# Fuad-HH/PumiUMTally

Hardware: AMD Instinct MI355X
Metric: particle-steps/sec (higher is better)
Workload: dtype fp64; 1 GPU; model=track-length-tally-walk, mesh_tets=998250, global_batch=10000000, particles_per_gpu=10000000, parallelism=dp1-replicated-mesh, nscores=1, comm=torch-rccl, ngroups=1, device=gpu, lost_particles=0

## Files before the change

### cpp/origin_delta_bench.cpp

```cpp
#include "core/origin_delta.h"

#include <hip/hip_runtime.h>

#include <algorithm>
#include <chrono>
#include <cstdio>
#include <cstdlib>
#include <cstring>
#include <memory>
#include <random>
#include <vector>

using namespace pumitally;

static double *pinned_doubles(int64_t count) {
  void *p = nullptr;
  if (hipHostMalloc(&p, count * sizeof(double), hipHostMallocDefault) !=
      hipSuccess) {
    std::fprintf(stderr, "hipHostMalloc failed\n");
    std::exit(2);
  }
  return (double *)p;
}

// ... 3 lines not shown
  double *ends[2] = {pinned_doubles(n * 3), pinned_doubles(n * 3)};
  double *alt = pinned_doubles(n * 3);
  std::mt19937_64 rng(1);
  std::uniform_real_distribution<double> u(0.0, 1.0);
  for (int64_t k = 0; k < n * 3; ++k) {
    ends[0][k] = u(rng);
    ends[1][k] = u(rng);
  }
  std::memcpy(alt, ends[0], n * 3 * sizeof(double));
  for (int64_t i = 0; i < n; ++i)
    if (rng() % 10 == 0) alt[i * 3 + 1] = u(rng);
  std::unique_ptr<double[]> shadow(new double[n * 3]);
  int64_t cap = 0;
  for (int nt : {1, 4, 8, 16})
    cap = std::max(cap, origin_delta_patch_capacity(n, nt));
  void *pi = nullptr, *px = nullptr;
  if (hipHostMalloc(&pi, cap * sizeof(int32_t), hipHostMallocDefault) !=
          hipSuccess ||
      hipHostMalloc(&px, cap * 3 * sizeof(double), hipHostMallocDefault) !=
          hipSuccess) {
    std::fprintf(stderr, "hipHostMalloc failed\n");
    return 2;
  }
  std::printf("n=%lld reps=%d (96 B/particle streamed, 120 B ordinary)\n",
              (long long)n, reps);
  for (int nt : {1, 4, 8, 16}) {
    OriginDeltaPool pool(nt);
    for (int nontemporal = 1; nontemporal >= 0; --nontemporal) {
      for (int frac10 = 0; frac10 < 2; ++frac10) {
        origin_delta_seed(pool, ends[0], shadow.get(), 0, n, nontemporal != 0);
        std::vector<double> ms;
        int64_t changed = 0;
        for (int r = 0; r < reps; ++r) {
          const double *origin =
              (frac10 && (r & 1) == 0) ? alt : ends[r & 1];
          const auto t0 = std::chrono::steady_clock::now();
          OriginDeltaResult res = origin_delta_pass(
              pool, origin, ends[(r + 1) & 1], shadow.get(), 0, n,
              (int32_t *)pi, (double *)px, nontemporal != 0);
          if (!res.overflow)
            origin_delta_compact(res, (int32_t *)pi, (double *)px);
          const auto t1 = std::chrono::steady_clock::now();
          ms.push_back(std::chrono::duration<double, std::milli>(t1 - t0)
                           .count());
          changed += res.changed;
        }
        std::sort(ms.begin(), ms.end());
        std::printf("threads=%2d stores=%-9s changed=%-4s  min %7.2f ms  "
                    "median %7.2f ms  (%.1f GB/s at median; changed/pass "
                    "%lld)\n",
                    nt, nontemporal ? "streaming" : "ordinary",
                    frac10 ? "~5%" : "0", ms.front(), ms[ms.size() / 2],
                    (nontemporal ? 96.0 : 120.0) * n / ms[ms.size() / 2] / 1e6,
                    (long long)(changed / reps));
      }
    }
  }
  return 0;
}
```

### csrc/core/engine.h

```cpp
#pragma once

#include "mesh.h"
#include "walk.h"

#include <cstdint>
#include <cstdlib>
#include <stdexcept>
#include <memory>
#include <string>
#include <vector>

namespace pumitally {

struct EngineStats {
  int64_t lost_particles = 0;
  int64_t moves = 0;
  int64_t relocated = 0;
  int64_t loose_localizations = 0;
  int64_t origins_elided = 0;
  int64_t origin_bytes_uploaded = 0;
  double origin_pass_seconds = 0.0;
  int64_t collisions_scored = 0;
  int64_t collision_misses = 0;
  int64_t tracks = 0;
  int64_t track_entries = 0;
  int64_t track_misses = 0;
};

constexpr int kMaxLostRecords = 16;

class Engine {
public:
  virtual ~Engine() = default;

  virtual int64_t num_particles() const = 0;
  virtual const Mesh &mesh() const = 0;

  virtual void copy_initial_position(const double *positions, int64_t n) = 0;

  virtual void move(const double *origin, const double *dest,
                    const int8_t *flying, const double *weights, int64_t n,
                    const uint16_t *groups = nullptr,
                    const double *responses = nullptr) = 0;

// ... 142 lines not shown
  };
  virtual bool device_mesh(DeviceMeshView *out) const {
    (void)out;
    return false;
  }

  int max_steps = 0;
  int ngroups = 1;
  int nscores = 1;

  bool reflective = false;

  bool linear = false;

  bool face_currents = false;

  bool collision_tallies = false;

  bool walk_fp32 = false;

  bool origin_elide = true;
  int origin_threads = 8;
  int64_t origin_chunk = 0;

protected:
  [[noreturn]] static void throw_not_linear() {
    throw std::runtime_error(
        "linear moment tallies are off: create the engine with linear=true");
  }
  [[noreturn]] static void throw_not_currents() {
    throw std::runtime_error(
        "face-current tallies are off: create the engine with currents=true");
  }
  [[noreturn]] static void throw_not_collisions() {
    throw std::runtime_error(
        "collision tallies are off: create the engine with collisions=true");
  }
};

inline bool default_walk_fp32() {
  const char *s = getenv("PUMITALLY_WALK");
  return s && std::string(s) == "fp32";
}

inline bool default_origin_elide() {
  const char *s = getenv("PUMITALLY_ORIGIN_ELIDE");
  return !s || atoi(s) != 0;
}

inline int default_origin_threads() {
  const char *s = getenv("PUMITALLY_ORIGIN_THREADS");
  const int k = s ? atoi(s) : 8;
  return k < 1 ? 1 : (k > 16 ? 16 : k);
}

inline int64_t default_origin_chunk() {
  const char *s = getenv("PUMITALLY_ORIGIN_CHUNK");
  const int64_t c = s ? (int64_t)atoll(s) : 0;
  return c < 0 ? 0 : c;
}

inline bool default_reflective() {
  const char *s = getenv("PUMITALLY_BC");
  return s && std::string(s) == "reflective";
}

inline double loc_tol_rel() {
  const char *s = getenv("PUMITALLY_LOC_TOL");
  return s ? atof(s) : 1e-10;
}
// ... 28 lines not shown
```

### csrc/core/origin_delta.cpp

```cpp
#include "origin_delta.h"

#include <algorithm>
#include <atomic>
#include <cstring>

#if defined(__SSE2__) && !defined(__HIP_DEVICE_COMPILE__)
#include <emmintrin.h>
#define PT_HAVE_STREAM_STORE 1
#else
#define PT_HAVE_STREAM_STORE 0
#endif

namespace pumitally {

int origin_delta_clamp_threads(int requested) {
  return std::max(1, std::min(requested, kOriginDeltaMaxThreads));
}

OriginDeltaPool::OriginDeltaPool(int nthreads)
    : nthreads_(origin_delta_clamp_threads(nthreads)) {
  for (int t = 1; t < nthreads_; ++t)
    threads_.emplace_back([this, t] { worker(t); });
}

// ... 90 lines not shown
        pidx[count] = (int32_t)i;
        pxyz[count * 3] = o[0];
        pxyz[count * 3 + 1] = o[1];
        pxyz[count * 3 + 2] = o[2];
      }
      ++count;
    }
    const double *d = dest + i * 3;
    store_bits<NT>(s, load_bits(d));
    store_bits<NT>(s + 1, load_bits(d + 1));
    store_bits<NT>(s + 2, load_bits(d + 2));
  }
  if (NT) store_fence();
  return count;
}

template <bool NT>
void copy_part(const double *dest, double *shadow, int64_t lo, int64_t hi) {
  for (int64_t k = lo * 3; k < hi * 3; ++k)
    store_bits<NT>(shadow + k, load_bits(dest + k));
  if (NT) store_fence();
}

}

int64_t origin_delta_block(int64_t len, int nthreads) {
  const int64_t t = origin_delta_clamp_threads(nthreads);
  const int64_t b = (len + 4 * t - 1) / (4 * t);
  return std::max<int64_t>(1, std::min(b, kMaxBlock));
}

int64_t origin_delta_patch_capacity(int64_t len, int nthreads) {
  if (len <= 0) return 0;
  const int64_t block = origin_delta_block(len, nthreads);
  const int64_t full = len / block, tail = len % block;
  return full * seg_capacity(block) + (tail ? seg_capacity(tail) : 0);
}

OriginDeltaResult origin_delta_pass(OriginDeltaPool &pool,
                                    const double *origin, const double *dest,
                                    double *shadow, int64_t lo, int64_t hi,
                                    int32_t *patch_idx, double *patch_xyz,
                                    bool nontemporal) {
  OriginDeltaResult r;
  const int64_t len = hi - lo;
  if (len <= 0) return r;
  r.block = origin_delta_block(len, pool.nthreads());
  r.nsegs = (len + r.block - 1) / r.block;
  r.seg_off.resize(r.nsegs);
  r.seg_cap.resize(r.nsegs);
  r.seg_count.assign(r.nsegs, 0);
  for (int64_t b = 0; b < r.nsegs; ++b) {
    const int64_t blen = std::min(r.block, len - b * r.block);
    r.seg_off[b] = b * seg_capacity(r.block);
    r.seg_cap[b] = seg_capacity(blen);
  }
  std::atomic<int64_t> next{0};
  const std::function<void(int)> job = [&](int) {
    for (;;) {
      const int64_t b = next.fetch_add(1, std::memory_order_relaxed);
      if (b >= r.nsegs) return;
      const int64_t a = lo + b * r.block;
      const int64_t e = std::min(hi, a + r.block);
      int32_t *pi = patch_idx + r.seg_off[b];
      double *px = patch_xyz + r.seg_off[b] * 3;
      r.seg_count[b] =
          nontemporal
              ? delta_part<true>(origin, dest, shadow, a, e, pi, px,
                                 r.seg_cap[b])
              : delta_part<false>(origin, dest, shadow, a, e, pi, px,
                                  r.seg_cap[b]);
    }
  };
  pool.run(job);
  for (int64_t b = 0; b < r.nsegs; ++b) {
    r.changed += r.seg_count[b];
    if (r.seg_count[b] > r.seg_cap[b]) r.overflow = true;
  }
  return r;
}

void origin_delta_compact(const OriginDeltaResult &r, int32_t *patch_idx,
                          double *patch_xyz) {
  int64_t out = 0;
  for (int64_t b = 0; b < r.nsegs; ++b) {
    const int64_t cnt = r.seg_count[b];
    if (cnt && r.seg_off[b] != out) {
      std::memmove(patch_idx + out, patch_idx + r.seg_off[b],
                   cnt * sizeof(int32_t));
      std::memmove(patch_xyz + out * 3, patch_xyz + r.seg_off[b] * 3,
                   cnt * 3 * sizeof(double));
    }
    out += cnt;
  }
}

void origin_delta_seed(OriginDeltaPool &pool, const double *dest,
                       double *shadow, int64_t lo, int64_t hi,
                       bool nontemporal) {
  const int64_t len = hi - lo;
  if (len <= 0) return;
// ... 20 lines not shown
```

### csrc/core/origin_delta.h

```cpp
#pragma once

#include <condition_variable>
#include <cstdint>
#include <functional>
#include <mutex>
#include <thread>
#include <vector>

namespace pumitally {

constexpr int kOriginDeltaMaxThreads = 16;

int origin_delta_clamp_threads(int requested);

class OriginDeltaPool {
public:
  explicit OriginDeltaPool(int nthreads);
  ~OriginDeltaPool();
  OriginDeltaPool(const OriginDeltaPool &) = delete;
  OriginDeltaPool &operator=(const OriginDeltaPool &) = delete;

  int nthreads() const { return nthreads_; }
  void run(const std::function<void(int)> &f);

// ... 9 lines not shown
  int pending_ = 0;
  bool stop_ = false;
};

struct OriginDeltaResult {
  int64_t block = 0;
  int64_t nsegs = 0;
  std::vector<int64_t> seg_off, seg_cap;
  std::vector<int64_t> seg_count;
  int64_t changed = 0;
  bool overflow = false;
};

int64_t origin_delta_block(int64_t len, int nthreads);

int64_t origin_delta_patch_capacity(int64_t len, int nthreads);

OriginDeltaResult origin_delta_pass(OriginDeltaPool &pool,
                                    const double *origin, const double *dest,
                                    double *shadow, int64_t lo, int64_t hi,
                                    int32_t *patch_idx, double *patch_xyz,
                                    bool nontemporal = false);

void origin_delta_compact(const OriginDeltaResult &r, int32_t *patch_idx,
                          double *patch_xyz);

void origin_delta_seed(OriginDeltaPool &pool, const double *dest,
                       double *shadow, int64_t lo, int64_t hi,
                       bool nontemporal = false);

}
```

### csrc/hip/engine_gpu.hip

```cpp
#include "../core/engine.h"
#include "../core/origin_delta.h"
#include "../core/tally_sink.h"
#include "../core/track.h"
#include "../core/walk.h"
#include "hip_util.h"

#include <hip/hip_runtime.h>
#include <hipcub/hipcub.hpp>

#include <algorithm>
#include <type_traits>
#include <array>
#include <chrono>
#include <cstdio>
#include <cstdlib>
#include <cstring>
#include <memory>
#include <stdexcept>
#include <string>
#include <vector>

namespace pumitally {

namespace {
// ... 670 lines not shown

int grid_blocks(int64_t work) {
  int64_t blocks = (work + kBlock - 1) / kBlock;
  if (blocks > grid_cap()) blocks = grid_cap();
  return (int)((blocks + 7) / 8 * 8);
}

class GpuEngine final : public Engine {
public:
  GpuEngine(Mesh mesh, int64_t n, int device, int groups, int scores,
            bool lin, bool cur, bool coll)
      : mesh_(std::move(mesh)), n_(n) {
    ngroups = groups < 1 ? 1 : groups;
    nscores = scores < 1 ? 1 : scores;
    linear = lin;
    face_currents = cur;
    collision_tallies = coll;
    PT_HIP_CHECK(hipSetDevice(device));
    device_ = device;
    s_copy_.create();
    s_comp_.create();
    for (auto &ev : copy_ev_) ev.create();
    for (auto &ev : kernels_done_) ev.create();
    if (collision_tallies) {
      s_score_.create();
      score_copied_.create();
      score_done_.create();
    }

    d_planes_ = upload(mesh_.planes);
    d_planes32_ = upload(mesh_.planes32);
    d_nbr_ = upload(mesh_.nbr);
    d_cell_start_ = upload(mesh_.grid.cell_start);
    d_cell_tets_.allocate(mesh_.grid.cell_tets.size() + 1);
    PT_HIP_CHECK(hipMemcpy(d_cell_tets_, mesh_.grid.cell_tets.data(),
                           mesh_.grid.cell_tets.size() * sizeof(int32_t),
                           hipMemcpyHostToDevice));
    d_face_bc_ = upload(mesh_.face_bc_bits);
    if (mesh_.has_periodic()) {
      d_pidx_ = upload(mesh_.periodic_idx);
      d_pelem_ = upload(mesh_.periodic_elem);
      d_pshift_ = upload(mesh_.periodic_shift);
    }
    grid_view_ = GridView{mesh_.grid.nx, mesh_.grid.ny, mesh_.grid.nz,
                          mesh_.grid.lo,  mesh_.grid.inv_h,
                          d_cell_start_,  d_cell_tets_};
// ... 13 lines not shown
      mesh_.build_inv_heights();
      d_inv_h_ = upload(mesh_.inv_heights);
      d_moments_.allocate(fsz_ * 4);
      PT_HIP_CHECK(hipMemset(d_moments_, 0, fsz_ * 4 * sizeof(double)));
    }
    if (face_currents) {
      d_cur_.allocate(fsz_ * 4);
      PT_HIP_CHECK(hipMemset(d_cur_, 0, fsz_ * 4 * sizeof(double)));
      cur_keyed_ = currents_keyed_agg() && mesh_.nelems < ((int64_t)1 << 29);
    }
    if (collision_tallies) {
      d_coll_.allocate(fsz_);
      PT_HIP_CHECK(hipMemset(d_coll_, 0, fsz_ * sizeof(double)));
      d_coll_counts_.allocate(2);
      PT_HIP_CHECK(
          hipMemset(d_coll_counts_, 0, 2 * sizeof(unsigned long long)));
      coll_agg_ = collisions_run_agg();
    }
    PT_HIP_CHECK(hipMemset(d_lost_, 0, sizeof(unsigned long long)));
    PT_HIP_CHECK(hipMemset(d_loose_, 0, sizeof(unsigned long long)));
    PT_HIP_CHECK(
        hipMemset(d_lostrec_, 0, kMaxLostRecords * 4 * sizeof(double)));

    for (int p = 0; p < 2; ++p) {
      d_origin_[p].allocate(n_ * 3);
      d_dest_[p].allocate(n_ * 3);
      d_flying_[p].allocate(n_);
      d_weights_[p].allocate(n_);
      if (ngroups > 1) d_groups_[p].allocate(n_);
    }

    sort_every_ = sort_every();
    if (sort_every_ > 0) {
      d_keys_.allocate(n_);
      d_keys2_.allocate(n_);
      d_vals_.allocate(n_);
      d_order_.allocate(n_);
      d_pos2_.allocate(n_ * 3);
      d_elem2_.allocate(n_);
      d_esc2_.allocate(n_);
      d_s2c2_.allocate(n_);
      size_t bytes = 0;
      PT_HIP_CHECK(hipcub::DeviceRadixSort::SortPairs(
          nullptr, bytes, d_keys_.get(), d_keys2_.get(), d_vals_.get(),
          d_order_.get(), (int)n_, 0, 64, s_comp_));
      sorttmp_bytes_ = bytes;
      d_sorttmp_.allocate(bytes ? bytes : 1);
      const Vec3 ext = mesh_.bbox_hi - mesh_.bbox_lo;
      sort_scale_ = Vec3{ext.x > 0 ? 2097151.0 / ext.x : 0.0,
                         ext.y > 0 ? 2097151.0 / ext.y : 0.0,
                         ext.z > 0 ? 2097151.0 / ext.z : 0.0};
    }

    loc_tol_ = loc_tol_rel() * norm(mesh_.bbox_hi - mesh_.bbox_lo);
    walk_fp32 = default_walk_fp32();
    reflective = default_reflective();
    origin_elide = default_origin_elide();
    origin_threads = default_origin_threads();
    origin_chunk = default_origin_chunk();
    const Vec3 c0 = mesh_.nelems > 0 ? mesh_.centroid(0) : Vec3{0, 0, 0};
    k_init_particles<<<grid_blocks(n_), kBlock, 0, s_comp_>>>(
        d_pos_, d_elem_, d_escaped_, d_s2c_, n_, c0.x, c0.y, c0.z);
    PT_HIP_CHECK(hipGetLastError());
    PT_HIP_CHECK(hipStreamSynchronize(s_comp_));
  }

  ~GpuEngine() override {
    (void)hipSetDevice(device_);
    (void)hipDeviceSynchronize();
  }

  int64_t num_particles() const override { return n_; }
  const Mesh &mesh() const override { return mesh_; }

  void copy_initial_position(const double *p, int64_t n) override {
    check_n(n);
    PT_HIP_CHECK(hipSetDevice(device_));
    sync();
    stage(p, n * 3 * sizeof(double), d_origin_[0], s_copy_);
    PT_HIP_CHECK(hipStreamSynchronize(s_copy_));
    k_iota<<<grid_blocks(n_), kBlock, 0, s_comp_>>>(d_s2c_, n_);
    k_locate<<<grid_blocks(n_), kBlock, 0, s_comp_>>>(
        d_planes_, grid_view_, d_origin_[0], d_pos_, d_elem_, d_escaped_,
        d_loose_, n_, loc_tol_);
    PT_HIP_CHECK(hipGetLastError());
    if (sort_every_ > 0) spatial_sort();
    moves_since_sort_ = 0;
    PT_HIP_CHECK(hipStreamSynchronize(s_comp_));
  }

  void move(const double *origin, const double *dest, const int8_t *flying,
            const double *weights, int64_t n,
            const uint16_t *groups = nullptr,
            const double *responses = nullptr) override {
    check_n(n);
    PT_HIP_CHECK(hipSetDevice(device_));
    const int steps = max_steps > 0 ? max_steps : default_max_steps(mesh_);
    const int p = (int)(parity_++ & 1);
    PT_HIP_CHECK(hipStreamWaitEvent(s_copy_, kernels_done_[p], 0));
    if (responses && !d_resp_[p]) d_resp_[p].allocate(n_ * nscores);
    const bool probe = origin && origin_elide && n > 0 && elide_skip_ == 0;
    if (probe && shadow_valid_) {
      stage_elided(p, origin, dest, flying, weights, groups, responses, n);
    } else {
      if (origin) {
        stage(origin, n * 3 * sizeof(double), d_origin_[p], s_copy_);
        stats_.origin_bytes_uploaded += n * 3 * (int64_t)sizeof(double);
      }
      stage_inputs(p, dest, flying, weights, groups, responses, n);
      shadow_valid_ = false;
      if (probe) {
        ensure_elide_host(n);
        const auto t0 = std::chrono::steady_clock::now();
        origin_delta_seed(*delta_pool_, dest, shadow_.get(), 0, n,
                          false);
        stats_.origin_pass_seconds += seconds_since(t0);
        shadow_valid_ = true;
      } else if (origin && origin_elide && elide_skip_ > 0) {
        --elide_skip_;
      }
    }
    PT_HIP_CHECK(hipEventRecord(copy_ev_[p], s_copy_));
    PT_HIP_CHECK(hipStreamWaitEvent(s_comp_, copy_ev_[p], 0));
    launch_move_chunks(origin ? d_origin_[p] : nullptr, d_dest_[p],
                       d_flying_[p], d_weights_[p],
                       groups ? d_groups_[p] : nullptr,
                       responses ? d_resp_[p] : nullptr, n, steps);
    PT_HIP_CHECK(hipEventRecord(kernels_done_[p], s_comp_));
    maybe_resort();
    PT_HIP_CHECK(hipStreamSynchronize(s_copy_));
    stats_.moves++;
  }

  void move_device(const double *d_origin, const double *d_dest,
                   const int8_t *d_flying, const double *d_weights, int64_t n,
                   const uint16_t *d_groups = nullptr,
                   const double *d_responses = nullptr) override {
    check_n(n);
    PT_HIP_CHECK(hipSetDevice(device_));
    const int steps = max_steps > 0 ? max_steps : default_max_steps(mesh_);
    launch_move_chunks(d_origin, d_dest, d_flying, d_weights, d_groups,
                       d_responses, n, steps);
    maybe_resort();
    stats_.moves++;
  }

  void score_collisions(const int8_t *active, const double *weights,
                        int64_t n, const uint16_t *groups = nullptr,
                        const double *responses = nullptr) override {
    if (!collision_tallies) throw_not_collisions();
    check_n(n);
// ... 497 lines not shown
    PT_HIP_CHECK(hipMemcpy(d_elem_, elem, n * sizeof(int32_t), hipMemcpyHostToDevice));
    PT_HIP_CHECK(hipMemcpy(d_escaped_, escaped, n, hipMemcpyHostToDevice));
    moves_since_sort_ = sort_every_;
  }

  void synchronize() override { sync(); }

  bool device_mesh(DeviceMeshView *out) const override {
    out->planes = d_planes_;
    out->nbr = d_nbr_;
    out->grid = grid_view_;
    out->stream = (void *)s_comp_;
    return true;
  }

private:
  void check_n(int64_t n) const {
    if (n != n_) throw std::runtime_error("particle count mismatch");
  }

  void sync() const {
    PT_HIP_CHECK(hipStreamSynchronize(s_copy_));
    PT_HIP_CHECK(hipStreamSynchronize(s_comp_));
  }

  void stage(const void *src, size_t bytes, void *dst, hipStream_t s) {
    PT_HIP_CHECK(hipMemcpyAsync(dst, src, bytes, hipMemcpyHostToDevice, s));
  }

  void stage_inputs(int p, const double *dest, const int8_t *flying,
                    const double *weights, const uint16_t *groups,
                    const double *responses, int64_t n) {
    stage(dest, n * 3 * sizeof(double), d_dest_[p], s_copy_);
    stage(flying, n * sizeof(int8_t), d_flying_[p], s_copy_);
    stage(weights, n * sizeof(double), d_weights_[p], s_copy_);
    if (groups && d_groups_[p])
      stage(groups, n * sizeof(uint16_t), d_groups_[p], s_copy_);
    if (responses)
      stage(responses, n * nscores * sizeof(double), d_resp_[p], s_copy_);
  }

  static constexpr int kElideBackoffFirst = 16;
  static constexpr int kElideBackoffMax = 256;

  static double seconds_since(std::chrono::steady_clock::time_point t0) {
    return std::chrono::duration<double>(std::chrono::steady_clock::now() -
                                         t0)
        .count();
  }

  int64_t elide_chunk(int64_t n) const {
    if (origin_chunk > 0) return std::max<int64_t>(origin_chunk, 64);
    return std::max<int64_t>((int64_t)262144, (n + 1) / 2);
  }

  void ensure_elide_host(int64_t n) {
    const int want = origin_delta_clamp_threads(origin_threads);
    if (!delta_pool_ || delta_pool_->nthreads() != want)
      delta_pool_ = std::make_unique<OriginDeltaPool>(want);
    if (!shadow_) shadow_.reset(new double[n * 3]);
  }

  void ensure_patch(int64_t need) {
    if (need <= patch_cap_) return;
    PT_HIP_CHECK(hipStreamSynchronize(s_copy_));
    patch_cap_ = 0;
    h_patch_idx_.reset();
    h_patch_xyz_.reset();
    d_patch_idx_.reset();
    d_patch_xyz_.reset();
    h_patch_idx_.allocate(need);
    h_patch_xyz_.allocate(need * 3);
    d_patch_idx_.allocate(need);
    d_patch_xyz_.allocate(need * 3);
    patch_cap_ = need;
  }

  void stage_elided(int p, const double *origin, const double *dest,
                    const int8_t *flying, const double *weights,
                    const uint16_t *groups, const double *responses,
                    int64_t n) {
    ensure_elide_host(n);
    const int nthreads = delta_pool_->nthreads();
    const int64_t chunk = elide_chunk(n);
    int64_t need = 0;
    for (int64_t lo = 0; lo < n; lo += chunk)
      need += origin_delta_patch_capacity(std::min(chunk, n - lo), nthreads);
    ensure_patch(need);
    shadow_valid_ = false;
    k_copy_doubles<<<grid_blocks(n * 3 / 2), kBlock, 0, s_copy_>>>(
        d_dest_[p ^ 1], d_origin_[p], n * 3);
    PT_HIP_CHECK(hipGetLastError());
    stage_inputs(p, dest, flying, weights, groups, responses, n);
    int64_t region = 0, uploaded = 0;
    for (int64_t lo = 0; lo < n; lo += chunk) {
      const int64_t hi = std::min(n, lo + chunk);
      const int64_t len = hi - lo;
      const int64_t cap = origin_delta_patch_capacity(len, nthreads);
      if (region + cap > patch_cap_)
        throw std::runtime_error("origin elision: patch region overflow");
      int32_t *hidx = h_patch_idx_ + region;
      double *hxyz = h_patch_xyz_ + region * 3;
      const auto t0 = std::chrono::steady_clock::now();
      const OriginDeltaResult r = origin_delta_pass(
          *delta_pool_, origin, dest, shadow_.get(), lo, hi, hidx, hxyz,
          false);
      stats_.origin_pass_seconds += seconds_since(t0);
      if (r.overflow || r.changed * 2 > len) {
        stage(origin + lo * 3, len * 3 * sizeof(double),
              d_origin_[p] + lo * 3, s_copy_);
        uploaded += len;
      } else if (r.changed > 0) {
        origin_delta_compact(r, hidx, hxyz);
        stage(hidx, r.changed * sizeof(int32_t), d_patch_idx_ + region,
              s_copy_);
        stage(hxyz, r.changed * 3 * sizeof(double),
              d_patch_xyz_ + region * 3, s_copy_);
        k_scatter_origins<<<grid_blocks(r.changed), kBlock, 0, s_copy_>>>(
            d_patch_idx_ + region, d_patch_xyz_ + region * 3, d_origin_[p],
            r.changed);
        PT_HIP_CHECK(hipGetLastError());
        uploaded += r.changed;
      }
      region += cap;
    }
    stats_.origins_elided += n - uploaded;
    stats_.origin_bytes_uploaded += uploaded * 3 * (int64_t)sizeof(double);
    shadow_valid_ = true;
    if (uploaded * 2 > n) {
      elide_skip_ = elide_backoff_;
      elide_backoff_ = std::min(elide_backoff_ * 2, kElideBackoffMax);
    } else {
      elide_backoff_ = kElideBackoffFirst;
    }
  }

  void launch_walk_raw(int64_t n, const double *pos, const double *dest,
                       const int32_t *elem, const double *weights,
                       double *out_pos, int32_t *out_elem, int8_t *out_status,
                       const uint16_t *groups, const double *resp,
                       double *out_dest, const double *in_t,
                       const int32_t *in_prev, double *out_o, double *out_t,
                       int32_t *out_prev) {
    const int steps = max_steps > 0 ? max_steps : default_max_steps(mesh_);
    const auto kernel =
        linear ? (walk_fp32 ? k_walk_raw<true, true> : k_walk_raw<false, true>)
        : face_currents
            ? (walk_fp32 ? k_walk_raw<true, false, true>
                         : k_walk_raw<false, false, true>)
            : (walk_fp32 ? k_walk_raw<true> : k_walk_raw<false>);
    kernel<<<grid_blocks(n), kBlock, 0, s_comp_>>>(
        d_planes_, d_planes32_, d_nbr_, pos, dest, elem, weights, groups, resp,
        out_pos, out_elem, out_status, out_dest, d_flux_, d_lost_, d_lostrec_,
        n, steps, reflective, d_face_bc_, ngroups, mesh_.nelems, nscores,
        d_pidx_, d_pelem_, d_pshift_, in_t, in_prev, out_o, out_t, out_prev,
        d_inv_h_, d_moments_, d_cur_);
    PT_HIP_CHECK(hipGetLastError());
// ... 68 lines not shown

  template <class T>
  std::pair<std::vector<int32_t>, std::vector<T>> fetch(const T *dev,
                                                        int comps) const {
    sync();
    std::vector<int32_t> s2c(n_);
    std::vector<T> v(n_ * comps);
    PT_HIP_CHECK(hipMemcpy(s2c.data(), d_s2c_, n_ * sizeof(int32_t),
                           hipMemcpyDeviceToHost));
    PT_HIP_CHECK(hipMemcpy(v.data(), dev, n_ * comps * sizeof(T),
                           hipMemcpyDeviceToHost));
    return {std::move(s2c), std::move(v)};
  }

  Mesh mesh_;
  int64_t n_;
  int64_t fsz_ = 0;
  int device_ = 0;
  double loc_tol_ = 1e-12;
  int slices_ = 1;
  int sort_every_ = 0;
  int64_t moves_since_sort_ = 0;
  uint64_t parity_ = 0;
  Vec3 sort_scale_{0, 0, 0};

  std::unique_ptr<double[]> shadow_;
  bool shadow_valid_ = false;
  std::unique_ptr<OriginDeltaPool> delta_pool_;
  int64_t patch_cap_ = 0;
  int elide_skip_ = 0;
  int elide_backoff_ = kElideBackoffFirst;

  Stream s_copy_, s_comp_;
  std::array<Event, 2> copy_ev_;
  std::array<Event, 2> kernels_done_;
  Stream s_score_;
  Event score_copied_, score_done_;
  bool score_queued_ = false;

  PinnedBuffer<int32_t> h_patch_idx_;
  PinnedBuffer<double> h_patch_xyz_;
  DeviceBuffer<int32_t> d_patch_idx_;
  DeviceBuffer<double> d_patch_xyz_;

  DeviceBuffer<Plane> d_planes_;
  DeviceBuffer<Plane32> d_planes32_;
  DeviceBuffer<int32_t> d_nbr_, d_cell_start_, d_cell_tets_;
  GridView grid_view_{};

  DeviceBuffer<double> d_pos_;
  DeviceBuffer<int32_t> d_elem_;
  DeviceBuffer<uint8_t> d_escaped_;
  DeviceBuffer<int32_t> d_s2c_;
  DeviceBuffer<double> d_flux_;
  DeviceBuffer<unsigned long long> d_lost_, d_loose_;
  DeviceBuffer<double> d_lostrec_;
  DeviceBuffer<double> d_origin_[2], d_dest_[2], d_weights_[2], d_resp_[2];
  DeviceBuffer<int8_t> d_flying_[2];
  DeviceBuffer<uint16_t> d_groups_[2];
  DeviceBuffer<double> d_bsum_, d_bsq_;
  DeviceBuffer<double> d_inv_h_, d_moments_, d_msum_;
  DeviceBuffer<double> d_cur_, d_csum_, d_csq_;
  bool cur_keyed_ = false;
  DeviceBuffer<double> d_coll_, d_collsum_, d_collsq_;
  DeviceBuffer<unsigned long long> d_coll_counts_;
  bool coll_agg_ = true;
  DeviceBuffer<int8_t> sc_active_;
  DeviceBuffer<double> sc_weights_, sc_resp_;
  DeviceBuffer<uint16_t> sc_groups_;
  ScorePointsScratch sp_;
  DeviceBuffer<uint32_t> d_face_bc_;
  DeviceBuffer<int32_t> d_pidx_, d_pelem_;
  DeviceBuffer<double> d_pshift_;
  WalkRawScratch wr_;
  DeviceBuffer<int32_t> d_face_start_, d_face_list_;
  DeviceBuffer<unsigned long long> d_track_counts_;
  bool tracks_refused_ = false;
  TrackScratch tt_;
  int64_t nbatches_ = 0;

// ... 31 lines not shown
```

### csrc/pybind/module.cpp

```cpp
#include <pybind11/numpy.h>
#include <pybind11/pybind11.h>
#include <pybind11/stl.h>

#include "../api/PumiTally.h"
#include "../comm/comm.h"
#include "../core/engine.h"
#include "../core/partition_engine.h"

#include <hip/hip_runtime.h>

#include <cstdint>
#include <cstring>
#include <memory>
#include <thread>
#include <vector>

namespace py = pybind11;
using namespace pumitally;

namespace {

bool have_gpu() {
  int n = 0;
  if (hipGetDeviceCount(&n) != hipSuccess) {
// ... 683 lines not shown
          [](const PyEngine &e) { return e.eng->face_currents; })
      .def_property_readonly(
          "reflective", [](const PyEngine &e) { return e.eng->reflective; })
      .def_property_readonly("ngroups",
                             [](const PyEngine &e) { return e.eng->ngroups; })
      .def_property_readonly("nscores",
                             [](const PyEngine &e) { return e.eng->nscores; })
      .def_property_readonly("num_particles",
                             [](const PyEngine &e) { return e.eng->num_particles(); })
      .def_property_readonly("is_gpu", [](const PyEngine &e) { return e.gpu; })
      .def_property(
          "max_steps", [](const PyEngine &e) { return e.eng->max_steps; },
          [](PyEngine &e, int v) { e.eng->max_steps = v; })
      .def_property(
          "origin_elide", [](const PyEngine &e) { return e.eng->origin_elide; },
          [](PyEngine &e, bool v) { e.eng->origin_elide = v; })
      .def_property(
          "origin_threads",
          [](const PyEngine &e) { return e.eng->origin_threads; },
          [](PyEngine &e, int v) { e.eng->origin_threads = v; })
      .def_property(
          "origin_chunk", [](const PyEngine &e) { return e.eng->origin_chunk; },
          [](PyEngine &e, int64_t v) { e.eng->origin_chunk = v; })
      .def("copy_initial_position",
           [](PyEngine &e, py::array_t<double, py::array::c_style | py::array::forcecast> p) {
             if ((int64_t)p.size() != e.eng->num_particles() * 3)
               throw std::runtime_error("positions must have size 3*num_particles");
             e.eng->copy_initial_position(p.data(), e.eng->num_particles());
           })
      .def("move",
           [](PyEngine &e, py::array_t<double, py::array::c_style> origin,
              py::array_t<double, py::array::c_style> dest,
              py::array_t<int8_t, py::array::c_style> flying,
              py::array_t<double, py::array::c_style> weights,
              py::object groups, py::object responses) {
             const int64_t n = e.eng->num_particles();
             if ((int64_t)origin.size() != n * 3 || (int64_t)dest.size() != n * 3 ||
                 (int64_t)flying.size() != n || (int64_t)weights.size() != n)
               throw std::runtime_error("move: array size mismatch");
             const uint16_t *gp = nullptr;
             py::array_t<uint16_t, py::array::c_style | py::array::forcecast> garr;
             if (!groups.is_none()) {
               garr = groups.cast<py::array_t<uint16_t, py::array::c_style | py::array::forcecast>>();
               if ((int64_t)garr.size() != n)
                 throw std::runtime_error("move: groups size mismatch");
               gp = garr.data();
// ... 303 lines not shown
              py::array_t<int32_t, py::array::c_style | py::array::forcecast> elem,
              py::array_t<uint8_t, py::array::c_style | py::array::forcecast> escaped) {
             const int64_t n = e.eng->num_particles();
             if ((int64_t)pos.size() != n * 3 || (int64_t)elem.size() != n ||
                 (int64_t)escaped.size() != n)
               throw std::runtime_error("set_particle_state: size mismatch");
             e.eng->set_particle_state(pos.data(), elem.data(), escaped.data(), n);
           })
      .def("end_batch", [](PyEngine &e) { py::gil_scoped_release ng; e.eng->end_batch(); })
      .def("batch_sum", [](const PyEngine &e) { return vec_to_np(e.eng->batch_sum()); })
      .def("batch_sum_sq", [](const PyEngine &e) { return vec_to_np(e.eng->batch_sum_sq()); })
      .def_property_readonly("num_batches",
                             [](const PyEngine &e) { return e.eng->num_batches(); })
      .def("stats", [](const PyEngine &e) {
        const EngineStats &s = e.eng->stats();
        py::dict d;
        d["lost_particles"] = s.lost_particles;
        d["moves"] = s.moves;
        d["relocated"] = s.relocated;
        d["loose_localizations"] = s.loose_localizations;
        d["origins_elided"] = s.origins_elided;
        d["origin_bytes_uploaded"] = s.origin_bytes_uploaded;
        d["origin_pass_seconds"] = s.origin_pass_seconds;
        d["collisions_scored"] = s.collisions_scored;
        d["collision_misses"] = s.collision_misses;
        d["tracks"] = s.tracks;
        d["track_entries"] = s.track_entries;
        d["track_misses"] = s.track_misses;
        return d;
      })
      .def("lost_records", [](const PyEngine &e) {
        auto v = e.eng->lost_records();
        auto arr = vec_to_np(std::move(v));
        return arr.reshape({(py::ssize_t)(arr.size() / 4), (py::ssize_t)4});
      });

  py::class_<PumiTally>(m, "PumiTally")
      .def(py::init([](const std::string &mesh, int32_t n) {
        int argc = 0;
        char **argv = nullptr;
        return new PumiTally(mesh, n, argc, argv);
      }))
      .def("copy_initial_position",
           [](PumiTally &t, py::array_t<double, py::array::c_style | py::array::forcecast> p) {
             t.CopyInitialPosition((double *)p.data(), (int32_t)p.size());
           })
// ... 19 lines not shown
```

### pumiumtally_amd/__init__.py

```python
from __future__ import annotations

import os as _os

if _os.environ.get("PUMITALLY_NO_TORCH", "0") != "1":
    try:
        import torch as _torch
    except ImportError:
        pass


def _load_core():
    try:
        from . import _core
        return _core
    except ImportError as e:
        if _os.environ.get("PUMITALLY_AUTOBUILD", "1") == "1":
            from ._build import build
            build()
            from . import _core
            return _core
        raise ImportError(
            "pumiumtally_amd._core is not built. Run "
            "`python -m pumiumtally_amd._build` first."
        ) from e
# ... 84 lines not shown
    @property
    def origin_elide(self) -> bool:
        return self._eng.origin_elide

    @origin_elide.setter
    def origin_elide(self, v: bool) -> None:
        self._eng.origin_elide = bool(v)

    @property
    def origin_threads(self) -> int:
        return self._eng.origin_threads

    @origin_threads.setter
    def origin_threads(self, v: int) -> None:
        self._eng.origin_threads = int(v)

    @property
    def origin_chunk(self) -> int:
        return self._eng.origin_chunk

    @origin_chunk.setter
    def origin_chunk(self, v: int) -> None:
        self._eng.origin_chunk = int(v)

    def copy_initial_position(self, positions):
        self._eng.copy_initial_position(positions)

    def move(self, origin, dest, flying, weights, groups=None,
             responses=None):
        self._eng.move(origin, dest, flying, weights, groups, responses)

    def move_continue(self, dest, flying, weights, groups=None,
                      responses=None):
        self._eng.move_continue(dest, flying, weights, groups, responses)

    def move_from_device(self, dest, flying, weights, origin=None,
                         sync_torch=True, groups=None, responses=None):
        def ptr(t, dtype, numel):
            return _device_ptr(t, dtype, numel, "move_from_device")

        n = self.num_particles
        if sync_torch:
            _sync_torch()
        self._eng.move_device(
            ptr(origin, "<f8", n * 3), ptr(dest, "<f8", n * 3),
            ptr(flying, "|i1", n), ptr(weights, "<f8", n),
# ... 432 lines not shown
```

Before: 1.445 billion particle-steps/s.

## Skip origin copy kernel when unchanged; add echo and owned-block origin elision modes

Rotates three device dest buffers so that, when no origin patches are needed, the walk reads origins in place from the previous step's dest buffer instead of launching a device copy kernel. It also adds two opt-in modes. One echoes device dest back to pinned host memory in slices and compares against it, so the host shadow copy write is dropped. The other uses owned-block work stealing for the host delta pass. The default path gains the copy-skip and extra buffer rotation, at the cost of an extra n*3 device buffer and more event synchronisation.

```diff
diff --git a/cpp/origin_delta_bench.cpp b/cpp/origin_delta_bench.cpp
--- a/cpp/origin_delta_bench.cpp
+++ b/cpp/origin_delta_bench.cpp
@@ -49,37 +49,63 @@
     std::fprintf(stderr, "hipHostMalloc failed\n");
     return 2;
   }
-  std::printf("n=%lld reps=%d (96 B/particle streamed, 120 B ordinary)\n",
+  std::printf("n=%lld reps=%d (96 B/particle streamed, 120 B ordinary, 48 B "
+              "compare only)\n",
               (long long)n, reps);
+  double *echoed = pinned_doubles(n * 3);
   for (int nt : {1, 4, 8, 16}) {
     OriginDeltaPool pool(nt);
-    for (int nontemporal = 1; nontemporal >= 0; --nontemporal) {
-      for (int frac10 = 0; frac10 < 2; ++frac10) {
-        origin_delta_seed(pool, ends[0], shadow.get(), 0, n, nontemporal != 0);
-        std::vector<double> ms;
-        int64_t changed = 0;
-        for (int r = 0; r < reps; ++r) {
-          const double *origin =
-              (frac10 && (r & 1) == 0) ? alt : ends[r & 1];
-          const auto t0 = std::chrono::steady_clock::now();
-          OriginDeltaResult res = origin_delta_pass(
-              pool, origin, ends[(r + 1) & 1], shadow.get(), 0, n,
-              (int32_t *)pi, (double *)px, nontemporal != 0);
-          if (!res.overflow)
-            origin_delta_compact(res, (int32_t *)pi, (double *)px);
-          const auto t1 = std::chrono::steady_clock::now();
-          ms.push_back(std::chrono::duration<double, std::milli>(t1 - t0)
-                           .count());
-          changed += res.changed;
+    for (int pass = 0; pass < 3; ++pass) {
+      for (int nontemporal = (pass == 0 ? 1 : 0); nontemporal >= 0;
+           --nontemporal) {
+        for (int frac10 = 0; frac10 < 2; ++frac10) {
+          if (pass == 1)
+            origin_delta_seed_owned(pool, ends[0], shadow.get(), 0, n);
+          else if (pass == 0)
+            origin_delta_seed(pool, ends[0], shadow.get(), 0, n,
+                              nontemporal != 0);
+          std::vector<double> ms;
+          int64_t changed = 0;
+          for (int r = 0; r < reps; ++r) {
+            const double *origin =
+                (frac10 && (r & 1) == 0) ? alt : ends[r & 1];
+            const double *dest = ends[(r + 1) & 1];
+            if (pass == 2)
+              std::memcpy(echoed, ends[r & 1], n * 3 * sizeof(double));
+            const auto t0 = std::chrono::steady_clock::now();
+            OriginDeltaResult res =
+                pass == 2   ? origin_delta_compare(pool, origin, echoed, 0, n,
+                                                   (int32_t *)pi, (double *)px)
+                : pass == 1 ? origin_delta_pass_owned(
+                                  pool, origin, dest, shadow.get(), 0, n,
+                                  (int32_t *)pi, (double *)px)
+                            : origin_delta_pass(
+                                  pool, origin, dest, shadow.get(), 0, n,
+                                  (int32_t *)pi, (double *)px,
+                                  nontemporal != 0);
+            if (!res.overflow)
+              origin_delta_compact(res, (int32_t *)pi, (double *)px);
+            const auto t1 = std::chrono::steady_clock::now();
+            ms.push_back(
+                std::chrono::duration<double, std::milli>(t1 - t0).count());
+            changed += res.changed;
+          }
+          std::sort(ms.begin(), ms.end());
+          const double bytes = pass == 2 ? 48.0 : nontemporal ? 96.0 : 120.0;
+          std::printf("threads=%2d pass=%-7s stores=%-9s changed=%-4s  min "
+                      "%7.2f ms  median %7.2f ms  (%.1f GB/s at median; "
+                      "changed/pass %lld)\n",
+                      nt,
+                      pass == 2   ? "compare"
+                      : pass == 1 ? "owned"
+                                  : "shared",
+                      pass == 2     ? "none"
+                      : nontemporal ? "streaming"
+                                    : "ordinary",
+                      frac10 ? "~5%" : "0", ms.front(), ms[ms.size() / 2],
+                      bytes * n / ms[ms.size() / 2] / 1e6,
+                      (long long)(changed / reps));
         }
-        std::sort(ms.begin(), ms.end());
-        std::printf("threads=%2d stores=%-9s changed=%-4s  min %7.2f ms  "
-                    "median %7.2f ms  (%.1f GB/s at median; changed/pass "
-                    "%lld)\n",
-                    nt, nontemporal ? "streaming" : "ordinary",
-                    frac10 ? "~5%" : "0", ms.front(), ms[ms.size() / 2],
-                    (nontemporal ? 96.0 : 120.0) * n / ms[ms.size() / 2] / 1e6,
-                    (long long)(changed / reps));
       }
     }
   }
diff --git a/csrc/core/engine.h b/csrc/core/engine.h
--- a/csrc/core/engine.h
+++ b/csrc/core/engine.h
@@ -20,6 +20,8 @@
   int64_t origins_elided = 0;
   int64_t origin_bytes_uploaded = 0;
   double origin_pass_seconds = 0.0;
+  int64_t origin_copy_kernels = 0;
+  double origin_echo_wait_seconds = 0.0;
   int64_t collisions_scored = 0;
   int64_t collision_misses = 0;
   int64_t tracks = 0;
@@ -208,6 +210,9 @@
   bool origin_elide = true;
   int origin_threads = 8;
   int64_t origin_chunk = 0;
+  bool origin_echo = false;
+  int origin_slices = 4;
+  bool origin_owned = false;
 
 protected:
   [[noreturn]] static void throw_not_linear() {
@@ -232,6 +237,22 @@
 inline bool default_origin_elide() {
   const char *s = getenv("PUMITALLY_ORIGIN_ELIDE");
   return !s || atoi(s) != 0;
+}
+
+inline bool default_origin_echo() {
+  const char *s = getenv("PUMITALLY_ORIGIN_ECHO");
+  return s && atoi(s) != 0;
+}
+
+inline bool default_origin_owned() {
+  const char *s = getenv("PUMITALLY_ORIGIN_OWNED");
+  return s && atoi(s) != 0;
+}
+
+inline int default_origin_slices() {
+  const char *s = getenv("PUMITALLY_ORIGIN_SLICES");
+  const int k = s ? atoi(s) : 4;
+  return k < 1 ? 1 : (k > 8 ? 8 : k);
 }
 
 inline int default_origin_threads() {
diff --git a/csrc/core/origin_delta.cpp b/csrc/core/origin_delta.cpp
--- a/csrc/core/origin_delta.cpp
+++ b/csrc/core/origin_delta.cpp
@@ -136,30 +136,44 @@
   if (NT) store_fence();
 }
 
-}
-
-int64_t origin_delta_block(int64_t len, int nthreads) {
-  const int64_t t = origin_delta_clamp_threads(nthreads);
-  const int64_t b = (len + 4 * t - 1) / (4 * t);
-  return std::max<int64_t>(1, std::min(b, kMaxBlock));
-}
-
-int64_t origin_delta_patch_capacity(int64_t len, int nthreads) {
-  if (len <= 0) return 0;
-  const int64_t block = origin_delta_block(len, nthreads);
-  const int64_t full = len / block, tail = len % block;
-  return full * seg_capacity(block) + (tail ? seg_capacity(tail) : 0);
-}
-
-OriginDeltaResult origin_delta_pass(OriginDeltaPool &pool,
-                                    const double *origin, const double *dest,
-                                    double *shadow, int64_t lo, int64_t hi,
-                                    int32_t *patch_idx, double *patch_xyz,
-                                    bool nontemporal) {
+constexpr int64_t kCompareTile = 64;
+
+inline uint64_t xor_or(const double *a, const double *b, int64_t nw) {
+  uint64_t acc = 0;
+  for (int64_t k = 0; k < nw; ++k) acc |= load_bits(a + k) ^ load_bits(b + k);
+  return acc;
+}
+
+int64_t compare_part(const double *origin, const double *shadow, int64_t lo,
+                     int64_t hi, int32_t *pidx, double *pxyz, int64_t cap) {
+  int64_t count = 0;
+  for (int64_t t = lo; t < hi; t += kCompareTile) {
+    const int64_t te = std::min(hi, t + kCompareTile);
+    if (!xor_or(origin + t * 3, shadow + t * 3, (te - t) * 3)) continue;
+    for (int64_t i = t; i < te; ++i) {
+      const double *o = origin + i * 3;
+      const double *s = shadow + i * 3;
+      const uint64_t diff = (load_bits(o) ^ load_bits(s)) |
+                            (load_bits(o + 1) ^ load_bits(s + 1)) |
+                            (load_bits(o + 2) ^ load_bits(s + 2));
+      if (diff) {
+        if (count < cap) {
+          pidx[count] = (int32_t)i;
+          pxyz[count * 3] = o[0];
+          pxyz[count * 3 + 1] = o[1];
+          pxyz[count * 3 + 2] = o[2];
+        }
+        ++count;
+      }
+    }
+  }
+  return count;
+}
+
+OriginDeltaResult segment_layout(int64_t len, int nthreads) {
   OriginDeltaResult r;
-  const int64_t len = hi - lo;
   if (len <= 0) return r;
-  r.block = origin_delta_block(len, pool.nthreads());
+  r.block = origin_delta_block(len, nthreads);
   r.nsegs = (len + r.block - 1) / r.block;
   r.seg_off.resize(r.nsegs);
   r.seg_cap.resize(r.nsegs);
@@ -169,6 +183,63 @@
     r.seg_off[b] = b * seg_capacity(r.block);
     r.seg_cap[b] = seg_capacity(blen);
   }
+  return r;
+}
+
+template <class Body>
+void run_blocks_owned(OriginDeltaPool &pool, int64_t nblocks, Body body) {
+  struct alignas(64) Cursor {
+    std::atomic<int64_t> next{0};
+    int64_t end = 0;
+  };
+  const int nt = pool.nthreads();
+  std::vector<Cursor> cur(nt);
+  for (int t = 0; t < nt; ++t) {
+    cur[t].next.store(nblocks * t / nt, std::memory_order_relaxed);
+    cur[t].end = nblocks * (t + 1) / nt;
+  }
+  const std::function<void(int)> job = [&](int t) {
+    for (int k = 0; k < nt; ++k) {
+      Cursor &c = cur[(t + k) % nt];
+      for (;;) {
+        const int64_t b = c.next.fetch_add(1, std::memory_order_relaxed);
+        if (b >= c.end) break;
+        body(b);
+      }
+    }
+  };
+  pool.run(job);
+}
+
+void sum_segments(OriginDeltaResult &r) {
+  for (int64_t b = 0; b < r.nsegs; ++b) {
+    r.changed += r.seg_count[b];
+    if (r.seg_count[b] > r.seg_cap[b]) r.overflow = true;
+  }
+}
+
+}
+
+int64_t origin_delta_block(int64_t len, int nthreads) {
+  const int64_t t = origin_delta_clamp_threads(nthreads);
+  const int64_t b = (len + 4 * t - 1) / (4 * t);
+  return std::max<int64_t>(1, std::min(b, kMaxBlock));
+}
+
+int64_t origin_delta_patch_capacity(int64_t len, int nthreads) {
+  if (len <= 0) return 0;
+  const int64_t block = origin_delta_block(len, nthreads);
+  const int64_t full = len / block, tail = len % block;
+  return full * seg_capacity(block) + (tail ? seg_capacity(tail) : 0);
+}
+
+OriginDeltaResult origin_delta_pass(OriginDeltaPool &pool,
+                                    const double *origin, const double *dest,
+                                    double *shadow, int64_t lo, int64_t hi,
+                                    int32_t *patch_idx, double *patch_xyz,
+                                    bool nontemporal) {
+  OriginDeltaResult r = segment_layout(hi - lo, pool.nthreads());
+  if (r.nsegs == 0) return r;
   std::atomic<int64_t> next{0};
   const std::function<void(int)> job = [&](int) {
     for (;;) {
@@ -187,10 +258,62 @@
     }
   };
   pool.run(job);
-  for (int64_t b = 0; b < r.nsegs; ++b) {
-    r.changed += r.seg_count[b];
-    if (r.seg_count[b] > r.seg_cap[b]) r.overflow = true;
-  }
+  sum_segments(r);
+  return r;
+}
+
+OriginDeltaResult origin_delta_pass_owned(OriginDeltaPool &pool,
+                                          const double *origin,
+                                          const double *dest, double *shadow,
+                                          int64_t lo, int64_t hi,
+                                          int32_t *patch_idx,
+                                          double *patch_xyz) {
+  OriginDeltaResult r = segment_layout(hi - lo, pool.nthreads());
+  if (r.nsegs == 0) return r;
+  run_blocks_owned(pool, r.nsegs, [&](int64_t b) {
+    const int64_t a = lo + b * r.block;
+    const int64_t e = std::min(hi, a + r.block);
+    r.seg_count[b] = delta_part<false>(origin, dest, shadow, a, e,
+                                       patch_idx + r.seg_off[b],
+                                       patch_xyz + r.seg_off[b] * 3,
+                                       r.seg_cap[b]);
+  });
+  sum_segments(r);
+  return r;
+}
+
+void origin_delta_seed_owned(OriginDeltaPool &pool, const double *dest,
+                             double *shadow, int64_t lo, int64_t hi) {
+  const int64_t len = hi - lo;
+  if (len <= 0) return;
+  const int64_t block = origin_delta_block(len, pool.nthreads());
+  run_blocks_owned(pool, (len + block - 1) / block, [&](int64_t b) {
+    const int64_t a = lo + b * block;
+    copy_part<false>(dest, shadow, a, std::min(hi, a + block));
+  });
+}
+
+OriginDeltaResult origin_delta_compare(OriginDeltaPool &pool,
+                                       const double *origin,
+                                       const double *shadow, int64_t lo,
+                                       int64_t hi, int32_t *patch_idx,
+                                       double *patch_xyz) {
+  OriginDeltaResult r = segment_layout(hi - lo, pool.nthreads());
+  if (r.nsegs == 0) return r;
+  std::atomic<int64_t> next{0};
+  const std::function<void(int)> job = [&](int) {
+    for (;;) {
+      const int64_t b = next.fetch_add(1, std::memory_order_relaxed);
+      if (b >= r.nsegs) return;
+      const int64_t a = lo + b * r.block;
+      const int64_t e = std::min(hi, a + r.block);
+      r.seg_count[b] =
+          compare_part(origin, shadow, a, e, patch_idx + r.seg_off[b],
+                       patch_xyz + r.seg_off[b] * 3, r.seg_cap[b]);
+    }
+  };
+  pool.run(job);
+  sum_segments(r);
   return r;
 }
 
diff --git a/csrc/core/origin_delta.h b/csrc/core/origin_delta.h
--- a/csrc/core/origin_delta.h
+++ b/csrc/core/origin_delta.h
@@ -55,6 +55,21 @@
                                     int32_t *patch_idx, double *patch_xyz,
                                     bool nontemporal = false);
 
+OriginDeltaResult origin_delta_pass_owned(OriginDeltaPool &pool,
+                                          const double *origin,
+                                          const double *dest, double *shadow,
+                                          int64_t lo, int64_t hi,
+                                          int32_t *patch_idx,
+                                          double *patch_xyz);
+void origin_delta_seed_owned(OriginDeltaPool &pool, const double *dest,
+                             double *shadow, int64_t lo, int64_t hi);
+
+OriginDeltaResult origin_delta_compare(OriginDeltaPool &pool,
+                                       const double *origin,
+                                       const double *shadow, int64_t lo,
+                                       int64_t hi, int32_t *patch_idx,
+                                       double *patch_xyz);
+
 void origin_delta_compact(const OriginDeltaResult &r, int32_t *patch_idx,
                           double *patch_xyz);
 
diff --git a/csrc/hip/engine_gpu.hip b/csrc/hip/engine_gpu.hip
--- a/csrc/hip/engine_gpu.hip
+++ b/csrc/hip/engine_gpu.hip
@@ -716,6 +716,9 @@
     s_comp_.create();
     for (auto &ev : copy_ev_) ev.create();
     for (auto &ev : kernels_done_) ev.create();
+    for (auto &ev : dest_read_) ev.create();
+    for (auto &ev : echo_done_) ev.create();
+    for (auto &ev : slice_up_) ev.create();
     if (collision_tallies) {
       s_score_.create();
       score_copied_.create();
@@ -775,9 +778,9 @@
     PT_HIP_CHECK(
         hipMemset(d_lostrec_, 0, kMaxLostRecords * 4 * sizeof(double)));
 
+    for (auto &d : d_dest_) d.allocate(n_ * 3);
     for (int p = 0; p < 2; ++p) {
       d_origin_[p].allocate(n_ * 3);
-      d_dest_[p].allocate(n_ * 3);
       d_flying_[p].allocate(n_);
       d_weights_[p].allocate(n_);
       if (ngroups > 1) d_groups_[p].allocate(n_);
@@ -811,6 +814,9 @@
     origin_elide = default_origin_elide();
     origin_threads = default_origin_threads();
     origin_chunk = default_origin_chunk();
+    origin_echo = default_origin_echo();
+    origin_slices = default_origin_slices();
+    origin_owned = default_origin_owned();
     const Vec3 c0 = mesh_.nelems > 0 ? mesh_.centroid(0) : Vec3{0, 0, 0};
     k_init_particles<<<grid_blocks(n_), kBlock, 0, s_comp_>>>(
         d_pos_, d_elem_, d_escaped_, d_s2c_, n_, c0.x, c0.y, c0.z);
@@ -850,36 +856,60 @@
     PT_HIP_CHECK(hipSetDevice(device_));
     const int steps = max_steps > 0 ? max_steps : default_max_steps(mesh_);
     const int p = (int)(parity_++ & 1);
+    const int b = (int)(dest_rot_++ % kDestBuffers);
     PT_HIP_CHECK(hipStreamWaitEvent(s_copy_, kernels_done_[p], 0));
+    PT_HIP_CHECK(hipStreamWaitEvent(s_copy_, dest_read_[b], 0));
+    PT_HIP_CHECK(hipStreamWaitEvent(s_copy_, echo_done_[b], 0));
     if (responses && !d_resp_[p]) d_resp_[p].allocate(n_ * nscores);
     const bool probe = origin && origin_elide && n > 0 && elide_skip_ == 0;
-    if (probe && shadow_valid_) {
-      stage_elided(p, origin, dest, flying, weights, groups, responses, n);
+    const double *d_org = origin ? d_origin_[p].get() : nullptr;
+    int in_place = -1;
+    if (probe && shadow_buf_ >= 0 && shadow_echoed_ == origin_echo) {
+      const int prev = shadow_buf_;
+      if (!stage_elided(p, b, prev, origin, dest, flying, weights, groups,
+                        responses, n)) {
+        d_org = d_dest_[prev];
+        in_place = prev;
+      }
     } else {
       if (origin) {
         stage(origin, n * 3 * sizeof(double), d_origin_[p], s_copy_);
         stats_.origin_bytes_uploaded += n * 3 * (int64_t)sizeof(double);
       }
-      stage_inputs(p, dest, flying, weights, groups, responses, n);
-      shadow_valid_ = false;
+      shadow_buf_ = -1;
+      stage_inputs(p, b, dest, flying, weights, groups, responses, n,
+                   probe && origin_echo);
       if (probe) {
-        ensure_elide_host(n);
-        const auto t0 = std::chrono::steady_clock::now();
-        origin_delta_seed(*delta_pool_, dest, shadow_.get(), 0, n,
-                          false);
-        stats_.origin_pass_seconds += seconds_since(t0);
-        shadow_valid_ = true;
+        if (!origin_echo) {
+          ensure_elide_host(n);
+          const auto t0 = std::chrono::steady_clock::now();
+          const int64_t chunk = elide_chunk(n);
+          for (int64_t lo = 0; lo < n; lo += chunk) {
+            const int64_t hi = std::min(n, lo + chunk);
+            if (origin_owned)
+              origin_delta_seed_owned(*delta_pool_, dest, shadow_.get(), lo,
+                                      hi);
+            else
+              origin_delta_seed(*delta_pool_, dest, shadow_.get(), lo, hi,
+                                false);
+          }
+          stats_.origin_pass_seconds += seconds_since(t0);
+        }
+        shadow_buf_ = b;
+        shadow_echoed_ = origin_echo;
       } else if (origin && origin_elide && elide_skip_ > 0) {
         --elide_skip_;
       }
     }
     PT_HIP_CHECK(hipEventRecord(copy_ev_[p], s_copy_));
     PT_HIP_CHECK(hipStreamWaitEvent(s_comp_, copy_ev_[p], 0));
-    launch_move_chunks(origin ? d_origin_[p] : nullptr, d_dest_[p],
-                       d_flying_[p], d_weights_[p],
+    launch_move_chunks(d_org, d_dest_[b], d_flying_[p], d_weights_[p],
                        groups ? d_groups_[p] : nullptr,
                        responses ? d_resp_[p] : nullptr, n, steps);
     PT_HIP_CHECK(hipEventRecord(kernels_done_[p], s_comp_));
+    PT_HIP_CHECK(hipEventRecord(dest_read_[b], s_comp_));
+    if (in_place >= 0)
+      PT_HIP_CHECK(hipEventRecord(dest_read_[in_place], s_comp_));
     maybe_resort();
     PT_HIP_CHECK(hipStreamSynchronize(s_copy_));
     stats_.moves++;
@@ -1423,16 +1453,40 @@
   void sync() const {
     PT_HIP_CHECK(hipStreamSynchronize(s_copy_));
     PT_HIP_CHECK(hipStreamSynchronize(s_comp_));
+    if (h_shadow_[0]) PT_HIP_CHECK(hipStreamSynchronize(s_echo_));
   }
 
   void stage(const void *src, size_t bytes, void *dst, hipStream_t s) {
     PT_HIP_CHECK(hipMemcpyAsync(dst, src, bytes, hipMemcpyHostToDevice, s));
   }
 
-  void stage_inputs(int p, const double *dest, const int8_t *flying,
+  void stage_inputs(int p, int b, const double *dest, const int8_t *flying,
                     const double *weights, const uint16_t *groups,
-                    const double *responses, int64_t n) {
-    stage(dest, n * 3 * sizeof(double), d_dest_[p], s_copy_);
+                    const double *responses, int64_t n, bool echo) {
+    if (echo) {
+      if (!h_shadow_[0]) {
+        s_echo_.create();
+        h_shadow_[0].allocate(n_ * 3);
+        h_shadow_[1].allocate(n_ * 3);
+      }
+      const int h = (int)(echo_seq_++ & 1);
+      const int nsl = std::max(1, std::min(origin_slices, kMaxSlices));
+      const int64_t len = std::max<int64_t>(1, (n + nsl - 1) / nsl);
+      int j = 0;
+      for (int64_t lo = 0; lo < n; lo += len, ++j) {
+        const size_t bytes = std::min(len, n - lo) * 3 * sizeof(double);
+        stage(dest + lo * 3, bytes, d_dest_[b] + lo * 3, s_copy_);
+        PT_HIP_CHECK(hipEventRecord(slice_up_[j], s_copy_));
+        PT_HIP_CHECK(hipStreamWaitEvent(s_echo_, slice_up_[j], 0));
+        PT_HIP_CHECK(hipMemcpyAsync(h_shadow_[h] + lo * 3,
+                                    d_dest_[b] + lo * 3, bytes,
+                                    hipMemcpyDeviceToHost, s_echo_));
+      }
+      PT_HIP_CHECK(hipEventRecord(echo_done_[b], s_echo_));
+      shadow_host_ = h;
+    } else {
+      stage(dest, n * 3 * sizeof(double), d_dest_[b], s_copy_);
+    }
     stage(flying, n * sizeof(int8_t), d_flying_[p], s_copy_);
     stage(weights, n * sizeof(double), d_weights_[p], s_copy_);
     if (groups && d_groups_[p])
@@ -1459,7 +1513,7 @@
     const int want = origin_delta_clamp_threads(origin_threads);
     if (!delta_pool_ || delta_pool_->nthreads() != want)
       delta_pool_ = std::make_unique<OriginDeltaPool>(want);
-    if (!shadow_) shadow_.reset(new double[n * 3]);
+    if (!origin_echo && !shadow_) shadow_.reset(new double[n * 3]);
   }
 
   void ensure_patch(int64_t need) {
@@ -1477,10 +1531,10 @@
     patch_cap_ = need;
   }
 
-  void stage_elided(int p, const double *origin, const double *dest,
-                    const int8_t *flying, const double *weights,
-                    const uint16_t *groups, const double *responses,
-                    int64_t n) {
+  bool stage_elided(int p, int b, int prev, const double *origin,
+                    const double *dest, const int8_t *flying,
+                    const double *weights, const uint16_t *groups,
+                    const double *responses, int64_t n) {
     ensure_elide_host(n);
     const int nthreads = delta_pool_->nthreads();
     const int64_t chunk = elide_chunk(n);
@@ -1488,11 +1542,24 @@
     for (int64_t lo = 0; lo < n; lo += chunk)
       need += origin_delta_patch_capacity(std::min(chunk, n - lo), nthreads);
     ensure_patch(need);
-    shadow_valid_ = false;
-    k_copy_doubles<<<grid_blocks(n * 3 / 2), kBlock, 0, s_copy_>>>(
-        d_dest_[p ^ 1], d_origin_[p], n * 3);
-    PT_HIP_CHECK(hipGetLastError());
-    stage_inputs(p, dest, flying, weights, groups, responses, n);
+    const bool echo = origin_echo;
+    const double *echoed = echo ? h_shadow_[shadow_host_].get() : nullptr;
+    shadow_buf_ = -1;
+    stage_inputs(p, b, dest, flying, weights, groups, responses, n, echo);
+    if (echo) {
+      const auto t0 = std::chrono::steady_clock::now();
+      PT_HIP_CHECK(hipEventSynchronize(echo_done_[prev]));
+      stats_.origin_echo_wait_seconds += seconds_since(t0);
+    }
+    bool copied = false;
+    const auto copy_previous = [&] {
+      if (copied) return;
+      k_copy_doubles<<<grid_blocks(n * 3 / 2), kBlock, 0, s_copy_>>>(
+          d_dest_[prev], d_origin_[p], n * 3);
+      PT_HIP_CHECK(hipGetLastError());
+      stats_.origin_copy_kernels++;
+      copied = true;
+    };
     int64_t region = 0, uploaded = 0;
     for (int64_t lo = 0; lo < n; lo += chunk) {
       const int64_t hi = std::min(n, lo + chunk);
@@ -1503,15 +1570,22 @@
       int32_t *hidx = h_patch_idx_ + region;
       double *hxyz = h_patch_xyz_ + region * 3;
       const auto t0 = std::chrono::steady_clock::now();
-      const OriginDeltaResult r = origin_delta_pass(
-          *delta_pool_, origin, dest, shadow_.get(), lo, hi, hidx, hxyz,
-          false);
+      const OriginDeltaResult r =
+          echo ? origin_delta_compare(*delta_pool_, origin, echoed, lo, hi,
+                                      hidx, hxyz)
+          : origin_owned
+              ? origin_delta_pass_owned(*delta_pool_, origin, dest,
+                                        shadow_.get(), lo, hi, hidx, hxyz)
+              : origin_delta_pass(*delta_pool_, origin, dest, shadow_.get(),
+                                  lo, hi, hidx, hxyz, false);
       stats_.origin_pass_seconds += seconds_since(t0);
       if (r.overflow || r.changed * 2 > len) {
+        copy_previous();
         stage(origin + lo * 3, len * 3 * sizeof(double),
               d_origin_[p] + lo * 3, s_copy_);
         uploaded += len;
       } else if (r.changed > 0) {
+        copy_previous();
         origin_delta_compact(r, hidx, hxyz);
         stage(hidx, r.changed * sizeof(int32_t), d_patch_idx_ + region,
               s_copy_);
@@ -1527,13 +1601,15 @@
     }
     stats_.origins_elided += n - uploaded;
     stats_.origin_bytes_uploaded += uploaded * 3 * (int64_t)sizeof(double);
-    shadow_valid_ = true;
+    shadow_buf_ = b;
+    shadow_echoed_ = echo;
     if (uploaded * 2 > n) {
       elide_skip_ = elide_backoff_;
       elide_backoff_ = std::min(elide_backoff_ * 2, kElideBackoffMax);
     } else {
       elide_backoff_ = kElideBackoffFirst;
     }
+    return copied;
   }
 
   void launch_walk_raw(int64_t n, const double *pos, const double *dest,
@@ -1648,10 +1724,14 @@
   int sort_every_ = 0;
   int64_t moves_since_sort_ = 0;
   uint64_t parity_ = 0;
+  uint64_t dest_rot_ = 0;
   Vec3 sort_scale_{0, 0, 0};
 
   std::unique_ptr<double[]> shadow_;
-  bool shadow_valid_ = false;
+  int shadow_buf_ = -1;
+  bool shadow_echoed_ = false;
+  int shadow_host_ = 0;
+  uint64_t echo_seq_ = 0;
   std::unique_ptr<OriginDeltaPool> delta_pool_;
   int64_t patch_cap_ = 0;
   int elide_skip_ = 0;
@@ -1660,12 +1740,18 @@
   Stream s_copy_, s_comp_;
   std::array<Event, 2> copy_ev_;
   std::array<Event, 2> kernels_done_;
+  static constexpr int kDestBuffers = 3;
+  static constexpr int kMaxSlices = 8;
+  Stream s_echo_;
+  std::array<Event, kDestBuffers> dest_read_, echo_done_;
+  std::array<Event, kMaxSlices> slice_up_;
   Stream s_score_;
   Event score_copied_, score_done_;
   bool score_queued_ = false;
 
   PinnedBuffer<int32_t> h_patch_idx_;
   PinnedBuffer<double> h_patch_xyz_;
+  PinnedBuffer<double> h_shadow_[2];
   DeviceBuffer<int32_t> d_patch_idx_;
   DeviceBuffer<double> d_patch_xyz_;
 
@@ -1681,7 +1767,8 @@
   DeviceBuffer<double> d_flux_;
   DeviceBuffer<unsigned long long> d_lost_, d_loose_;
   DeviceBuffer<double> d_lostrec_;
-  DeviceBuffer<double> d_origin_[2], d_dest_[2], d_weights_[2], d_resp_[2];
+  DeviceBuffer<double> d_origin_[2], d_dest_[kDestBuffers], d_weights_[2],
+      d_resp_[2];
   DeviceBuffer<int8_t> d_flying_[2];
   DeviceBuffer<uint16_t> d_groups_[2];
   DeviceBuffer<double> d_bsum_, d_bsq_;
diff --git a/csrc/pybind/module.cpp b/csrc/pybind/module.cpp
--- a/csrc/pybind/module.cpp
+++ b/csrc/pybind/module.cpp
@@ -729,6 +729,16 @@
       .def_property(
           "origin_chunk", [](const PyEngine &e) { return e.eng->origin_chunk; },
           [](PyEngine &e, int64_t v) { e.eng->origin_chunk = v; })
+      .def_property(
+          "origin_echo", [](const PyEngine &e) { return e.eng->origin_echo; },
+          [](PyEngine &e, bool v) { e.eng->origin_echo = v; })
+      .def_property(
+          "origin_owned", [](const PyEngine &e) { return e.eng->origin_owned; },
+          [](PyEngine &e, bool v) { e.eng->origin_owned = v; })
+      .def_property(
+          "origin_slices",
+          [](const PyEngine &e) { return e.eng->origin_slices; },
+          [](PyEngine &e, int v) { e.eng->origin_slices = v; })
       .def("copy_initial_position",
            [](PyEngine &e, py::array_t<double, py::array::c_style | py::array::forcecast> p) {
              if ((int64_t)p.size() != e.eng->num_particles() * 3)
@@ -1078,6 +1088,8 @@
         d["origins_elided"] = s.origins_elided;
         d["origin_bytes_uploaded"] = s.origin_bytes_uploaded;
         d["origin_pass_seconds"] = s.origin_pass_seconds;
+        d["origin_copy_kernels"] = s.origin_copy_kernels;
+        d["origin_echo_wait_seconds"] = s.origin_echo_wait_seconds;
         d["collisions_scored"] = s.collisions_scored;
         d["collision_misses"] = s.collision_misses;
         d["tracks"] = s.tracks;
diff --git a/pumiumtally_amd/__init__.py b/pumiumtally_amd/__init__.py
--- a/pumiumtally_amd/__init__.py
+++ b/pumiumtally_amd/__init__.py
@@ -130,6 +130,30 @@
     @origin_chunk.setter
     def origin_chunk(self, v: int) -> None:
         self._eng.origin_chunk = int(v)
+
+    @property
+    def origin_echo(self) -> bool:
+        return self._eng.origin_echo
+
+    @origin_echo.setter
+    def origin_echo(self, v: bool) -> None:
+        self._eng.origin_echo = bool(v)
+
+    @property
+    def origin_owned(self) -> bool:
+        return self._eng.origin_owned
+
+    @origin_owned.setter
+    def origin_owned(self, v: bool) -> None:
+        self._eng.origin_owned = bool(v)
+
+    @property
+    def origin_slices(self) -> int:
+        return self._eng.origin_slices
+
+    @origin_slices.setter
+    def origin_slices(self, v: int) -> None:
+        self._eng.origin_slices = int(v)
 
     def copy_initial_position(self, positions):
         self._eng.copy_initial_position(positions)
```

After: 1.433 billion particle-steps/s. No clear change (-0.9%).
